# themattinthehatt/behavenet

Hardware: AMD Instinct MI355X
Metric: AE training frames/sec (128x128x1, batch 256) (higher is better)
Workload: dtype f32; 1 GPU; configs[1]: conv AE default arch, 1x128x128 f32 frames resident in HBM, 12 latents, batch 256 (chunks 200+56), fwd+bwd+Adam(amsgrad)

## Files before the change

behavenet_amd/_hip.py:

```python

import ctypes
import os

import torch

_LIB_NAME = 'libbehavenet_hip.so'
_LIB_PATH = os.environ.get('BN_HIP_LIB') or os.path.join(
    os.path.dirname(os.path.abspath(__file__)), _LIB_NAME)
_lib = None

ACT_NONE, ACT_LRELU, ACT_SIGMOID = 0, 1, 2

PROF_NONE, PROF_CONV_FWD, PROF_CONV_BWD_D, PROF_CONV_BWD_W = 0, 1, 2, 3
PROF_CONVT_FWD, PROF_CONVT_BWD_D, PROF_CONVT_BWD_W, PROF_ADAM = 4, 5, 6, 7
PROF_LINEAR_FWD, PROF_LINEAR_BWD = 8, 9

_c_int, _c_float, _c_size_t, _c_void_p = ctypes.c_int, ctypes.c_float, ctypes.c_size_t, ctypes.c_void_p

_CONV_GEOM = [_c_int] * 12
_ACT_WS = [_c_int, _c_float, _c_void_p, _c_size_t, _c_void_p]

OP_CONV_FWD, OP_CONV_BWD_D, OP_CONV_BWD_W = 1, 2, 3
OP_CONVT_FWD, OP_CONVT_BWD_D, OP_CONVT_BWD_W = 4, 5, 6

# ... 30 lines not shown
    'bn_batchnorm_act_bwd': (
        _c_int, [_c_void_p] * 9 + [_c_int] * 6 + [_c_float, _c_void_p, _c_size_t, _c_void_p]),
    'bn_batchnorm_moment': (_c_int, [_c_void_p] * 3 + [_c_int] * 3 + [_c_void_p, _c_size_t, _c_void_p]),
    'bn_batchnorm_bwd_reduce': (
        _c_int, [_c_void_p] * 7 + [_c_int] * 4 + [_c_float, _c_void_p, _c_size_t, _c_void_p]),
    'bn_batchnorm_bwd_apply': (
        _c_int, [_c_void_p] * 9 + [_c_int] * 3 + [_c_float, _c_int, _c_float, _c_void_p]),
    'bn_maxpool2d_fwd': (_c_int, [_c_void_p] * 3 + [_c_int] * 9 + [_c_void_p]),
    'bn_maxpool2d_bwd': (_c_int, [_c_void_p] * 3 + [_c_int] * 9 + [_c_void_p]),
    'bn_maxpool2d_act_fwd': (_c_int, [_c_void_p] * 3 + [_c_int] * 4 + [ctypes.c_float, _c_void_p]),
    'bn_conv2d_pool2_act_fwd': (_c_int, [_c_void_p] * 5 + _CONV_GEOM + [_c_int, _c_float, _c_void_p]),
    'bn_conv2d_pool2_act_ok': (_c_int, _CONV_GEOM),
    'bn_conv2d_pool2_bwd_weight_ws_bytes': (_c_size_t, _CONV_GEOM),
    'bn_conv2d_pool2_bwd_weight': (
        _c_int, [_c_void_p] * 6 + _CONV_GEOM + [_c_int, _c_float, _c_int, _c_void_p, _c_size_t, _c_void_p]),
    'bn_maxpool2d_act_bwd': (_c_int, [_c_void_p] * 4 + [_c_int] * 4 + [ctypes.c_float, _c_void_p]),
    'bn_maxunpool2d_fwd': (_c_int, [_c_void_p] * 3 + [_c_int] * 3 + [_c_void_p]),
    'bn_maxunpool2d_fwd_k2': (_c_int, [_c_void_p] * 3 + [_c_int] * 3 + [_c_void_p]),
    'bn_maxunpool2d_bwd': (_c_int, [_c_void_p] * 3 + [_c_int] * 3 + [_c_void_p]),
    'bn_act_fwd': (_c_int, [_c_void_p] * 2 + [_c_size_t, _c_int, _c_float, _c_void_p]),
    'bn_act_bwd': (_c_int, [_c_void_p] * 3 + [_c_size_t, _c_int, _c_float, _c_void_p]),
    'bn_linear_ws_bytes': (_c_size_t, [_c_int] * 3),
    'bn_linear_fwd': (_c_int, [_c_void_p] * 4 + [_c_int] * 3 + [_c_void_p, _c_size_t, _c_void_p]),
    'bn_linear_bwd': (
        _c_int, [_c_void_p] * 5 + [_c_int, _c_float, _c_void_p, _c_void_p, _c_int] +
        [_c_int] * 3 + [_c_void_p, _c_size_t, _c_void_p]),
    'bn_sqerr_frame_sums': (_c_int, [_c_void_p] * 4 + [_c_int, _c_size_t, _c_void_p]),
    'bn_sqerr_bwd': (_c_int, [_c_void_p] * 4 + [_c_size_t, _c_float, _c_void_p, _c_void_p]),
    'bn_convT2d_fwd_sqerr_parts': (_c_int, _CONV_GEOM),
    'bn_convT2d_fwd_sqerr_ws_bytes': (_c_size_t, _CONV_GEOM + [_c_int]),
    'bn_convT2d_fwd_sqerr': (
        _c_int, [_c_void_p] * 8 + _CONV_GEOM + [_c_int, _c_float, _c_void_p, _c_size_t, _c_void_p]),
    'bn_scale_frames': (_c_int, [_c_void_p] * 4 + [_c_int, _c_size_t, _c_void_p]),
    'bn_reduce_sum': (_c_int, [_c_void_p] * 2 + [_c_size_t, _c_float, _c_void_p]),
    'bn_reparam_fwd': (_c_int, [_c_void_p] * 4 + [_c_size_t, _c_void_p]),
    'bn_kl_rows': (_c_int, [_c_void_p] * 3 + [_c_int, _c_int, _c_void_p]),
    'bn_reparam_bwd': (_c_int, [_c_void_p] * 4 + [_c_size_t, _c_void_p]),
    'bn_kl_bwd': (_c_int, [_c_void_p] * 4 + [_c_size_t, _c_float, _c_void_p, _c_void_p]),
    'bn_decomposed_kl_fwd': (_c_int, [_c_void_p] * 7 + [_c_int, _c_int, _c_void_p]),
    'bn_decomposed_kl_bwd': (_c_int, [_c_void_p] * 9 + [_c_int, _c_int, _c_void_p]),
    'bn_psvae_head_fwd': (_c_int, [_c_void_p] * 14 + [_c_int] * 3 + [_c_void_p]),
    'bn_psvae_head_combine': (
        _c_int, [_c_void_p] * 4 + [_c_int] + [_c_float] * 3 + [_c_int] + [_c_void_p] * 3),
    'bn_psvae_head_bwd': (
        _c_int, [_c_void_p] * 3 + [_c_int] + [_c_void_p] * 10 + [_c_float] + [_c_void_p] * 5 +
        [_c_int] * 4 + [_c_void_p]),
    'bn_adam_amsgrad_step': (
        _c_int, [_c_void_p] * 5 + [_c_size_t] + [_c_float] * 5 + [_c_int, _c_void_p]),
    'bn_u8_to_unit_float': (_c_int, [_c_void_p] * 2 + [_c_size_t, _c_void_p]),
    'bn_prof_select': (_c_int, [_c_int] * 3),
    'bn_prof_select_nth': (_c_int, [_c_int] * 4),
    'bn_prof_read': (_c_int, [ctypes.POINTER(ctypes.c_double), ctypes.POINTER(ctypes.c_long)]),
    'bn_prof_read_main': (_c_int, [ctypes.POINTER(ctypes.c_double), ctypes.POINTER(ctypes.c_long)]),
    'bn_prof_set_bracket': (_c_int, [_c_int]),
    'bn_prof_kernel_name': (ctypes.c_char_p, []),
    'bn_prof_dispatch_overhead_us': (ctypes.c_double, [_c_int, _c_void_p]),
}


class HipLibraryError(RuntimeError):
    pass


def lib_path():
    return _LIB_PATH

# ... 427 lines not shown

def convT2d_fwd_sqerr(x, w, b, target, mask, geom, act, slope, want_xhat):
    N, Ci, Hi, Wi, Co, R, S, st, ct, cl, Ho, Wo = geom
    lib = load()
    P = lib.bn_convT2d_fwd_sqerr_parts(*geom)
    if P <= 0:
        raise HipLibraryError('bn_convT2d_fwd_sqerr_parts: bad geometry %s' % (geom,))
    xhat = torch.empty((N, Co, Ho, Wo), dtype=torch.float32, device=x.device) if want_xhat \
        else None
    dpre = torch.empty((N, Co, Ho, Wo), dtype=torch.float32, device=x.device)
    part = torch.empty((N, P), dtype=torch.float32, device=x.device)
    nbytes = lib.bn_convT2d_fwd_sqerr_ws_bytes(*geom, int(want_xhat))
    ws = None
    if nbytes:
        ws = _arena(x.device, nbytes, 'fwd_sqerr')
    _check(lib.bn_convT2d_fwd_sqerr(
        _ptr(x, 'x'), _ptr(w, 'w'), _ptr(b, 'b', allow_none=True), _ptr(target, 'target'),
        _ptr(mask, 'mask', allow_none=True), _ptr(xhat, 'xhat', allow_none=True),
        _ptr(dpre, 'dpre'), _ptr(part, 'part'), *geom, act, slope, ws, nbytes, _stream()),
        'bn_convT2d_fwd_sqerr')
    return xhat, dpre, part


def scale_frames(t, frame_scale, group_scale=None, group_of_frame=None):
    N = t.shape[0]
    _check(load().bn_scale_frames(
        _ptr(t, 't'), _ptr(frame_scale, 'frame_scale'),
        _ptr(group_scale, 'group_scale', allow_none=True),
        _ptr(group_of_frame, 'group_of_frame', dtype=torch.int32, allow_none=True),
        N, t.numel() // N, _stream()), 'bn_scale_frames')
    return t


def reduce_sum(t, scale=1.0, out=None):
    if out is None:
        out = torch.empty((), dtype=torch.float32, device=t.device)
    _check(load().bn_reduce_sum(_ptr(t, 'in'), _ptr(out, 'out'), t.numel(), float(scale),
                                _stream()), 'bn_reduce_sum')
    return out


def reparam_fwd(mu, logvar, eps):
    z = torch.empty_like(mu)
    _check(load().bn_reparam_fwd(
        _ptr(mu, 'mu'), _ptr(logvar, 'logvar'), _ptr(eps, 'eps'), _ptr(z, 'z'), mu.numel(),
        _stream()), 'bn_reparam_fwd')
    return z


def kl_rows(mu, logvar):
    N, D = mu.shape
    out = torch.empty((N,), dtype=torch.float32, device=mu.device)
    _check(load().bn_kl_rows(_ptr(mu, 'mu'), _ptr(logvar, 'logvar'), _ptr(out, 'kl_rows'), N, D,
                             _stream()), 'bn_kl_rows')
    return out


DECOMPOSED_KL_MAX_D = 64


def _check_dkl_width(D):
    if D > DECOMPOSED_KL_MAX_D:
        raise ValueError('decomposed KL: %d latent dimensions, the kernels serve at most %d'
                         % (D, DECOMPOSED_KL_MAX_D))


# ... 224 lines not shown
```

behavenet_amd/csrc/bn_fast.h:

```cpp
#pragma once
#include "bn_common.h"

struct BnFastPlan {
    bool supported;
    const char* kernel_name;
    size_t ws_bytes;
    int variant;
    int a, b, c, d;
};

BnFastPlan bn_fast_down_plan(const BnGeom& g);
BnFastPlan bn_fast_up_plan(const BnGeom& g);
BnFastPlan bn_fast_wgrad_plan(const BnGeom& g);

int bn_launch_down_fast(const BnFastPlan& plan, const float* big, const float* w,
                        const float* bias, float* out, const float* dact_src, const BnGeom& g,
                        int act, int dact, float slope, void* ws, hipStream_t st);
int bn_launch_up_fast(const BnFastPlan& plan, const float* small, const float* w,
                      const float* bias, float* out, const float* dact_src, const BnGeom& g,
                      int act, int dact, float slope, void* ws, hipStream_t st);
int bn_launch_wgrad_fast(const BnFastPlan& plan, const float* small, const float* big, float* dw,
                         const BnGeom& g, int accumulate, void* ws, hipStream_t st,
                         float* db = nullptr, int bias_side = 0, bool* bias_done = nullptr);

// ... 20 lines not shown
                     const BnGeom& g, int accumulate, void* ws, hipStream_t st, float* db,
                     int bias_side, bool* bias_done);

BnFastPlan bn_s5_up_plan(const BnGeom& g);
BnFastPlan bn_s5_wgrad_plan(const BnGeom& g);
int bn_launch_up_s5(const float* small, const float* w, const float* bias, float* out,
                    const float* dact_src, const BnGeom& g, int act, int dact, float slope,
                    hipStream_t st);
int bn_launch_wgrad_s5(const float* small, const float* big, float* dw, const BnGeom& g,
                       int accumulate, hipStream_t st);

BnFastPlan bn_edge_wgrad_plan(const BnGeom& g);
int bn_launch_edge_wgrad(const BnFastPlan& plan, const float* small, const float* big, float* dw,
                         const BnGeom& g, int accumulate, void* ws, hipStream_t st,
                         float* db = nullptr, int bias_side = 0, bool* bias_done = nullptr);
bool bn_s1c1_ok(const BnGeom& g);
int bn_launch_s1c1(const float* big, const float* w, const float* bias, float* out, const float* dact_src,
                   const BnGeom& g, int act, int dact, float slope, hipStream_t st);
bool bn_s1in1_ok(const BnGeom& g);
int bn_launch_s1in1(const float* big, const float* w, const float* bias, float* out, const float* dact_src,
                    const BnGeom& g, int act, int dact, float slope, hipStream_t st);
BnFastPlan bn_edge_down_plan(const BnGeom& g);
const char* bn_edge_down_kernel_name(const BnGeom& g, int act, bool has_dact, bool u8);
const char* bn_edge_up_kernel_name(const BnGeom& g, bool loss);
int bn_launch_edge_down(const float* big, const float* w, const float* bias, float* out,
                        const float* dact_src, const BnGeom& g, int act, int dact, float slope,
                        hipStream_t st, const unsigned char* u8 = nullptr);
BnFastPlan bn_edge_up_plan(const BnGeom& g);
int bn_launch_edge_up(const float* small, const float* w, const float* bias, float* out,
                      const BnGeom& g, int act, float slope, hipStream_t st,
                      const float* target = nullptr, const float* mask = nullptr,
                      float* dpre = nullptr, float* partial = nullptr);
int bn_edge_up_parts_per_frame(const BnGeom& g);

bool bn_qgemm_supported(const BnGeom& g);
size_t bn_qgemm_ws_bytes(int role, const BnGeom& g);
int bn_launch_qgemm_down(const float* big, const float* w, const float* bias, float* out,
                         const float* dact_src, const BnGeom& g, int act, int dact, float slope,
                         void* ws, hipStream_t st);
int bn_launch_qgemm_up(const float* small, const float* w, const float* bias, float* out,
                       const float* dact_src, const BnGeom& g, int act, int dact, float slope,
                       void* ws, hipStream_t st);
int bn_launch_qgemm_wgrad(const float* small, const float* big, float* dw, const BnGeom& g,
                          int accumulate, void* ws, hipStream_t st);

bool bn_qg2_up_supported(const BnGeom& g, int act, int dact);
int bn_launch_qg2_up(const float* small, const float* w, const float* bias, float* out,
                     const float* dact_src, const BnGeom& g, int act, int dact, float slope,
                     hipStream_t st);
bool bn_qg2_wgrad_supported(const BnGeom& g);
int bn_launch_qg2_wgrad(const float* small, const float* big, float* dw, const BnGeom& g,
                        int accumulate, float* db, int bias_side, hipStream_t st);

bool bn_s5win_supported(const BnGeom& g);
size_t bn_s5win_ws_bytes(int role, const BnGeom& g);
int bn_launch_s5win_down(const float* big, const float* w, const float* bias, float* out,
                         const float* dact_src, const BnGeom& g, int act, int dact, float slope,
                         void* ws, hipStream_t st);
int bn_launch_s5win_up(const float* small, const float* w, const float* bias, float* out,
                       const float* dact_src, const BnGeom& g, int act, int dact, float slope,
                       hipStream_t st);
int bn_launch_s5win_wgrad(const float* small, const float* big, float* dw, const BnGeom& g,
                          int accumulate, hipStream_t st);

int bn_launch_split_epilogue(const float* part, const float* bias, float* out, const float* dact_src,
                             size_t total, int splits, int C, int npix, int act, int dact, float slope,
// ... 2 lines not shown
```

behavenet_amd/csrc/bn_launch.h:

```cpp
#pragma once
#include "bn_common.h"

struct GemmArgs {
    const float* A; long sai, sak;
    const float* B; long sbk, sbj;
    float* C; long sci, scj;
    int M, N, K;
    const float* bias_j;
    const float* dact_src;
    int dact; float slope;
    int accumulate;
    float* part;
    int kslice;
};

int bn_launch_down_generic(const float* big, const float* w, const float* bias, float* out,
                           const float* dact_src, const BnGeom& g, int act, int dact, float slope,
                           hipStream_t st);
int bn_launch_up_generic(const float* small, const float* w, const float* bias, float* out,
                         const float* dact_src, const BnGeom& g, int act, int dact, float slope,
                         hipStream_t st);
int bn_launch_wgrad_generic(const float* small, const float* big, float* dw, const BnGeom& g,
                            int accumulate, hipStream_t st);
size_t bn_channel_sum_ws_bytes(int N, int C, int npix);
int bn_launch_channel_sum(const float* t, float* db, int N, int C, int npix, int accumulate,
                          void* ws, size_t ws_bytes, hipStream_t st);

int bn_launch_gemm(const GemmArgs& a, hipStream_t st, void* ws = nullptr, size_t ws_bytes = 0);
size_t bn_gemm_ws_bytes(int M, int N, int K);
int bn_launch_col_sum(const float* dy, float* db, int M, int N, int accumulate, hipStream_t st);
int bn_launch_linear_jobs(const GemmArgs* g0, const GemmArgs* g1, const float* dy, float* db, int M,
                          int N, int accumulate, void* ws, size_t ws_bytes, hipStream_t st);
size_t bn_linear_jobs_ws_bytes(int M, int N, int K);

int bn_launch_act_fwd(const float* x, float* y, size_t n, int act, float slope, hipStream_t st);
int bn_launch_act_bwd(const float* dy, const float* y, float* dpre, size_t n, int act, float slope,
                      hipStream_t st);
int bn_launch_sqerr_frame_sums(const float* pred, const float* target, const float* mask,
                               float* frame_sums, int N, size_t D, hipStream_t st);
int bn_launch_sqerr_bwd(const float* pred, const float* target, const float* mask, float* dpred,
                        size_t n, float scale, const float* gscale, hipStream_t st);
int bn_launch_scale_frames(float* t, const float* frame_scale, const float* group_scale,
                           const int* group_of_frame, int N, size_t D, hipStream_t st);
int bn_launch_reduce_sum(const float* in, float* out, size_t n, float scale, hipStream_t st);
int bn_launch_reparam_fwd(const float* mu, const float* logvar, const float* eps, float* z,
                          size_t n, hipStream_t st);
int bn_launch_kl_rows(const float* mu, const float* logvar, float* kl_rows, int N, int D,
                      hipStream_t st);
int bn_launch_reparam_bwd(const float* dz, const float* z, const float* mu, float* dlogvar,
                          size_t n, hipStream_t st);
int bn_launch_kl_bwd(const float* mu, const float* logvar, float* dmu, float* dlogvar, size_t n,
                     float scale, const float* gscale, hipStream_t st);
int bn_launch_adam(float* p, const float* g, float* m, float* v, float* vmax, size_t n, float lr,
                   float b1, float b2, float eps, float wd, int step, hipStream_t st);
int bn_launch_u8_to_unit_float(const unsigned char* in, float* out, size_t n, hipStream_t st);

size_t bn_batchnorm_ws_bytes_impl(int N, int C);
int bn_launch_bn_stats(const float* x, float* mean, float* var, int N, int C, int HW, void* ws,
                       hipStream_t st);
// ... 89 lines not shown
```

behavenet_amd/csrc/capi.hip:

```cpp
#include <math.h>
#include <stdio.h>
#include <stdlib.h>
#include <string.h>
#include <hip/hip_ext.h>
#include "bn_common.h"
#include "bn_launch.h"
#include "bn_fast.h"

namespace {
struct ProfState {
    int family = BN_PROF_NONE;
    int C = 0, K = 0;
    static const int kMaxSlots = 2048;
    hipEvent_t ev[4 * kMaxSlots];
    bool taken[kMaxSlots], bracketed[kMaxSlots];
    int created = 0;
    int used = 0;
    double total_ms = 0.0, main_ms = 0.0;
    long launches = 0, main_launches = 0;
    bool bracket = true;
    int nth = -1, seen = 0;
    char kernel_name[96] = "";
} g_prof;

// ... 1551 lines not shown
    if (!x || !w || !target || !dpre || !part) return BN_E_BADARG;
    const BnGeom g = convT_geom(N, Ci, Hi, Wi, Co, R, S, stride, crop_t, crop_l, Ho, Wo);
    if (!bn_geom_ok(g)) return BN_E_BADARG;
    hipStream_t st = (hipStream_t)stream;
    if (fused_sqerr_fast(g)) {
        BnProfScope prof(BN_PROF_CONVT_FWD, g.Cs, g.Cb, bn_edge_up_kernel_name(g, true), st);
        return bn_launch_edge_up(x, w, b, xhat, g, act, slope, st, target, mask, dpre, part);
    }
    const size_t need = bn_convT2d_fwd_sqerr_ws_bytes(N, Ci, Hi, Wi, Co, R, S, stride, crop_t,
                                                      crop_l, Ho, Wo, xhat != nullptr);
    if (need && (!ws || ws_bytes < need)) return BN_E_WORKSPACE;
    const size_t n_out = (size_t)N * Co * Ho * Wo;
    const size_t conv_ws = need - (xhat ? 0 : n_out * sizeof(float));
    float* xh = xhat ? xhat : (float*)((char*)ws + conv_ws);
    int rc = run_up(BN_PROF_CONVT_FWD, x, w, b, xh, nullptr, g, act, BN_ACT_NONE, slope, ws,
                    conv_ws, st);
    if (rc) return rc;
    rc = bn_launch_sqerr_frame_sums(xh, target, mask, part, N, (size_t)Co * Ho * Wo, st);
    if (rc) return rc;
    rc = bn_launch_sqerr_bwd(xh, target, mask, dpre, n_out, 1.f, nullptr, st);
    if (rc) return rc;
    if (act != BN_ACT_NONE) rc = bn_launch_act_bwd(dpre, xh, dpre, n_out, act, slope, st);
    return rc;
}

extern "C" int bn_scale_frames(float* t, const float* frame_scale, const float* group_scale,
                               const int* group_of_frame, int N, size_t D, bn_stream_t stream) {
    if (!t || !frame_scale || N <= 0 || D == 0) return BN_E_BADARG;
    if ((group_scale == nullptr) != (group_of_frame == nullptr)) return BN_E_BADARG;
    return bn_launch_scale_frames(t, frame_scale, group_scale, group_of_frame, N, D,
                                  (hipStream_t)stream);
}

extern "C" int bn_reduce_sum(const float* in, float* out, size_t n, float scale,
                             bn_stream_t stream) {
    if (!in || !out) return BN_E_BADARG;
    return bn_launch_reduce_sum(in, out, n, scale, (hipStream_t)stream);
}

extern "C" int bn_reparam_fwd(const float* mu, const float* logvar, const float* eps, float* z,
                              size_t n, bn_stream_t stream) {
    if (!mu || !logvar || !eps || !z) return BN_E_BADARG;
    if (n == 0) return 0;
    return bn_launch_reparam_fwd(mu, logvar, eps, z, n, (hipStream_t)stream);
}

extern "C" int bn_kl_rows(const float* mu, const float* logvar, float* kl_rows, int N, int D,
                          bn_stream_t stream) {
    if (!mu || !logvar || !kl_rows || N <= 0 || D <= 0) return BN_E_BADARG;
    return bn_launch_kl_rows(mu, logvar, kl_rows, N, D, (hipStream_t)stream);
}

extern "C" int bn_reparam_bwd(const float* dz, const float* z, const float* mu, float* dlogvar,
                              size_t n, bn_stream_t stream) {
    if (!dz || !z || !mu || !dlogvar) return BN_E_BADARG;
    if (n == 0) return 0;
    return bn_launch_reparam_bwd(dz, z, mu, dlogvar, n, (hipStream_t)stream);
}

extern "C" int bn_kl_bwd(const float* mu, const float* logvar, float* dmu, float* dlogvar,
                         size_t n, float scale, const float* gscale, bn_stream_t stream) {
    if (!mu || !logvar || !dmu || !dlogvar) return BN_E_BADARG;
    if (n == 0) return 0;
    return bn_launch_kl_bwd(mu, logvar, dmu, dlogvar, n, scale, gscale, (hipStream_t)stream);
}

// ... 36 lines not shown
```

behavenet_amd/csrc/conv_edge.hip:

```cpp
#include <hip/hip_ext.h>
#include <stdlib.h>
#include "bn_common.h"
#include "bn_fast.h"
#include "bn_reduce.h"

typedef float floatx16 __attribute__((ext_vector_type(16)));

#define ED_THREADS 256
#define ED_OOB 0x7fffffff

__device__ __forceinline__ float ed_ld(__amdgpu_buffer_rsrc_t r, int byte_off) {
    return __builtin_bit_cast(float, __builtin_amdgcn_raw_buffer_load_b32(r, byte_off, 0, 0));
}

#define WC_ROWS 4
#define WC_W 64
#define WC_TPX (WC_ROWS * WC_W)
#define WC_SP (WC_TPX + 2)
#define WC_IH (2 * WC_ROWS + 3)
#define WC_RW (2 * WC_W + 4)
#define WC_KS (32 * WC_TPX / ED_THREADS)

#define WC_DECODE_GRID()                                                                    \
    int bch, bx, G;                                                                         \
    if (pair) {                                                                             \
        const int id = blockIdx.x, r = id >> 3;                                             \
        G = gridDim.x / g.Cb;                                                               \
        bch = r % g.Cb;                                                                     \
        bx = (r / g.Cb) * 8 + (id & 7);                                                     \
    } else {                                                                                \
        bch = blockIdx.y; bx = blockIdx.x; G = gridDim.x;                                   \
    }

template <int ST, bool VEC = false>
__global__ __launch_bounds__(ED_THREADS) void k_wgrad_c1(
    const float* __restrict__ small, const float* __restrict__ big, float* __restrict__ part,
// ... 1467 lines not shown
            ? launch_down_c1w<BN_ACT_LRELU>(big, w, bias, out, g, slope, st, e0, e1)
            : launch_down_c1w<BN_ACT_NONE>(big, w, bias, out, g, slope, st, e0, e1);
    if (variant == 3) variant = dact_src ? 1 : 0;
    if (variant == 2) {
        if (act == BN_ACT_LRELU && !dact_src)
            return launch_down_c1s<BN_ACT_LRELU, false, false, 4>(big, w, bias, out, nullptr, g, slope, st, e0, e1);
        if (!dact_src)
            return launch_down_c1s<BN_ACT_NONE, false, false, 4>(big, w, bias, out, nullptr, g, slope, st, e0, e1);
        return launch_down_c1s<BN_ACT_NONE, true, false, 4>(big, w, bias, out, dact_src, g, slope, st, e0, e1);
    }
    if (variant == 1) {
        if (act == BN_ACT_LRELU && !dact_src)
            return launch_down_c1s<BN_ACT_LRELU, false, false, 2>(big, w, bias, out, nullptr, g, slope, st, e0, e1);
        if (!dact_src)
            return launch_down_c1s<BN_ACT_NONE, false, false, 2>(big, w, bias, out, nullptr, g, slope, st, e0, e1);
        return launch_down_c1s<BN_ACT_NONE, true, false, 2>(big, w, bias, out, dact_src, g, slope, st, e0, e1);
    }
    const int units = g.N * (g.Hs / DC_ROWS);
    const dim3 grid(down_c1_grid(units));
    if (act == BN_ACT_LRELU && !dact_src) {
        hipExtLaunchKernelGGL((k_down_c1<BN_ACT_LRELU, false>), grid, dim3(64), 0, st, e0, e1, 0,
                              big, w, bias, out, dact_src, g, slope, units);
    } else if (act == BN_ACT_NONE && !dact_src) {
        hipExtLaunchKernelGGL((k_down_c1<BN_ACT_NONE, false>), grid, dim3(64), 0, st, e0, e1, 0,
                              big, w, bias, out, dact_src, g, slope, units);
    } else {
        hipExtLaunchKernelGGL((k_down_c1<BN_ACT_NONE, true>), grid, dim3(64), 0, st, e0, e1, 0,
                              big, w, bias, out, dact_src, g, slope, units);
    }
    BN_LAUNCH_CHECK();
    return 0;
}

#define UC_TH 8
#define UC_W 64
#define UC_PW (UC_W + 2)
#define UC_NPOS ((UC_TH + 2) * UC_PW)
#define UC_NBLK ((UC_NPOS + 31) / 32)
#define UC_DP (UC_NBLK * 32)
#define UC_LDS (25 * UC_DP * 4)

__global__ __launch_bounds__(ED_THREADS) void k_up_c1(
    const float* __restrict__ small, const float* __restrict__ w, const float* __restrict__ bias,
    float* __restrict__ out, BnGeom g, int act, float slope) {
    extern __shared__ __attribute__((aligned(16))) float dl[];
    const int tid = threadIdx.x, lane = tid & 63;
    const int wv = __builtin_amdgcn_readfirstlane(tid >> 6);
    const int li = lane & 31, kk = lane >> 5;
    const int tiles_per_frame = g.Hs / UC_TH;
    const int n = blockIdx.x / tiles_per_frame;
    const int a0 = (blockIdx.x - n * tiles_per_frame) * UC_TH;
    const int HWs = g.Hs * g.Ws;

    const __amdgpu_buffer_rsrc_t rs = __builtin_amdgcn_make_buffer_rsrc(
        (void*)small, 0, (int)((size_t)g.N * g.Cs * HWs * 4), 0x00020000);

    float av[16];
#pragma unroll
    for (int t = 0; t < 16; ++t) {
        const int c = 2 * t + kk;
        av[t] = (li < 25 && c < g.Cs) ? w[(c * g.Cb + blockIdx.y) * 25 + li] : 0.f;
    }

    for (int blk = wv; blk < UC_NBLK; blk += 4) {
        const int f = blk * 32 + li;
        const int py = f / UC_PW, px = f - py * UC_PW;
// ... 1006 lines not shown
```

behavenet_amd/csrc/conv_generic.hip:

```cpp
#include "bn_common.h"
#include "bn_launch.h"

#define GEN_THREADS 256
#define GEN_MT 8
#define GEN_MAXS 16

__global__ __launch_bounds__(GEN_THREADS) void k_down_generic(
    const float* __restrict__ big, const float* __restrict__ w, const float* __restrict__ bias,
    float* __restrict__ out, const float* __restrict__ dact_src, BnGeom g, int act, int dact,
    float slope) {
    const int pix = blockIdx.x * GEN_THREADS + threadIdx.x;
    const int npix = g.Hs * g.Ws;
    const int m0 = blockIdx.y * GEN_MT;
    const int n = blockIdx.z;
    if (pix >= npix) return;
    const int p = pix / g.Ws, q = pix - p * g.Ws;
    const int RS = g.R * g.S;
    float acc[GEN_MT];
#pragma unroll
    for (int j = 0; j < GEN_MT; ++j) acc[j] = 0.f;

    const int h0 = p * g.stride - g.pt, w0 = q * g.stride - g.pl;
    for (int c = 0; c < g.Cb; ++c) {
        const float* bp = big + ((size_t)n * g.Cb + c) * g.Hb * g.Wb;
// ... 192 lines not shown
    for (int n = n_beg; n < n_end; ++n) {
        const float* tp = t + ((size_t)n * C + c) * npix;
        if (vec) {
            const float4* t4 = reinterpret_cast<const float4*>(tp);
            for (int i = threadIdx.x; i < (npix >> 2); i += GEN_THREADS) {
                const float4 v = t4[i];
                acc += (v.x + v.y) + (v.z + v.w);
            }
        } else {
            for (int i = threadIdx.x; i < npix; i += GEN_THREADS) acc += tp[i];
        }
    }
    const float s = bn_block_reduce_256(acc, red);
    if (threadIdx.x == 0) part[(size_t)c * S + sp] = s;
}

__global__ __launch_bounds__(64) void k_channel_sum_final(const float* __restrict__ part, float* __restrict__ db,
                                                          int C, int S, int accumulate) {
    const int c = blockIdx.x;
    float v = 0.f;
    for (int s = threadIdx.x; s < S; s += 64) v += part[(size_t)c * S + s];
#pragma unroll
    for (int off = 32; off > 0; off >>= 1) v += __shfl_xor(v, off, 64);
    if (threadIdx.x == 0) db[c] = accumulate ? db[c] + v : v;
}

static int channel_sum_splits(int N, int C, int npix) {
    if ((long)N * npix < 8192) return 1;
    int s = 1024 / C;
    if (s > 256) s = 256;
    if (s > N) s = N;
    return s < 1 ? 1 : s;
}

size_t bn_channel_sum_ws_bytes(int N, int C, int npix) {
    const int s = channel_sum_splits(N, C, npix);
    return s > 1 ? (size_t)C * s * sizeof(float) : 0;
}

int bn_launch_channel_sum(const float* t, float* db, int N, int C, int npix, int accumulate,
                          void* ws, size_t ws_bytes, hipStream_t st) {
    const int S = channel_sum_splits(N, C, npix);
    if (S > 1 && ws && ws_bytes >= (size_t)C * S * sizeof(float)) {
        hipLaunchKernelGGL(k_channel_sum_part, dim3(C, S), dim3(GEN_THREADS), 0, st, t, (float*)ws,
                           N, C, npix, S);
        BN_LAUNCH_CHECK();
        hipLaunchKernelGGL(k_channel_sum_final, dim3(C), dim3(64), 0, st,
                           (const float*)ws, db, C, S, accumulate);
        BN_LAUNCH_CHECK();
        return 0;
    }
    hipLaunchKernelGGL(k_channel_sum, dim3(C), dim3(GEN_THREADS), 0, st, t, db, N, C, npix,
                       accumulate);
    BN_LAUNCH_CHECK();
    return 0;
}

#include "bn_reduce.h"
__global__ __launch_bounds__(1024) void k_sum_partials(const float* __restrict__ part,
                                                       float* __restrict__ out, int total,
                                                       int splits, int accumulate, int ab_elems,
                                                       int ntap, int row_len, int row_stride) {
    __shared__ float red[16][64];
    const int il = threadIdx.x & 63, zl = threadIdx.x >> 6;
    const int nz = blockDim.x >> 6;
    const int i = blockIdx.x * 64 + il;
// ... 66 lines not shown
```

behavenet_amd/hip_functions.py:

```python

import collections.abc
import os

import torch

from behavenet_amd import _hip

LRELU_SLOPE = 0.05

_direct_grads = False


class accumulate_into_param_grads(object):

    def __enter__(self):
        global _direct_grads
        self._prev = _direct_grads
        _direct_grads = True

    def __exit__(self, *exc):
        global _direct_grads
        _direct_grads = self._prev
        return False

# ... 360 lines not shown
            if i == 0 and h1 is not None:
                h = h1
            else:
                h = _fwd(layer, h, params[2 * i].detach(), params[2 * i + 1].detach(),
                         w5=taps[i] if taps else None)
            acts.append(h)
        if _sign_tap is not None:
            rec = _sign_tap.setdefault(id(plan), [[] for _ in plan])
            for i, layer in enumerate(plan):
                if layer.act == _hip.ACT_LRELU:
                    rec[i].append((acts[i + 1] > 0).cpu())
        ctx.plan = plan
        ctx.taps = taps
        ctx.need_dx = x.requires_grad
        ctx.param_refs = params
        _note_use(params, any(ctx.needs_input_grad[3:]))
        ctx.save_for_backward(*acts, *params[0::2])
        return h

    @staticmethod
    def backward(ctx, dout):
        plan = ctx.plan
        dout = dout.contiguous()
        top = plan[-1]
        if top.act != _hip.ACT_NONE:
            dpre = _hip.act_bwd(dout, ctx.saved_tensors[len(plan)], top.act, LRELU_SLOPE)
        else:
            dpre = dout
        dx, grads = _stack_backward(ctx, dpre, first_param=3)
        return (None, dx, None) + tuple(grads)


_DGRAD_FIRST = os.environ.get('BN_DGRAD_FIRST', '0') == '1'


def _stack_backward(ctx, dpre, first_param):
    plan = ctx.plan
    n_layers = len(plan)
    saved = ctx.saved_tensors
    acts, weights = saved[:n_layers + 1], saved[n_layers + 1:2 * n_layers + 1]
    n = dpre.shape[0]
    grads = [None] * (2 * n_layers)
    taps = getattr(ctx, 'taps', None)
    tail = []
    for i in range(n_layers - 1, -1, -1):
        layer = plan[i]
        g = layer.geom(n)
        w = weights[i]
        x_in = acts[i]
        if x_in.dtype == torch.uint8:
            x_in = _hip.u8_to_unit_float(x_in) \
                if ctx.needs_input_grad[first_param + 2 * i] else None
        need_w = ctx.needs_input_grad[first_param + 2 * i]
        need_b = ctx.needs_input_grad[first_param + 1 + 2 * i]
        dpre_below = None
        if i > 0 and min(plan[i - 1].cin, plan[i - 1].cout) <= 4 and _DGRAD_FIRST:
            dact_src, dact = acts[i], plan[i - 1].act
            bwd_data = _hip.conv2d_bwd_data if layer.kind == 'conv' else _hip.convT2d_bwd_data
            dpre_below = bwd_data(dpre, w, g, dact_src, dact, LRELU_SLOPE, w5=taps[i] if taps else None)
        if need_w:
            gw = _grad_buffer(ctx.param_refs[2 * i])
            gb = _grad_buffer(ctx.param_refs[2 * i + 1]) if need_b else None
            direct = gw is not None and (gb is not None or not need_b)
            if direct:
                dw, db = gw, gb
            else:
                dw = torch.empty_like(w)
                db = torch.empty((layer.cout,), dtype=w.dtype, device=w.device) if need_b \
                    else None
            wgrad = _hip.conv2d_bwd_weight if layer.kind == 'conv' else _hip.convT2d_bwd_weight
            side = _side_stream(w.device) if (direct and _use_side_stream) else None
            if side is not None and not ctx.need_dx and i < _tail_on_main:
                tail.append(((wgrad, x_in, dpre, dw, db, g), ctx.param_refs[2 * i:2 * i + 2]))
            elif side is not None:
                main = torch.cuda.current_stream(w.device)
                ev = torch.cuda.Event()
                ev.record(main)
                with torch.cuda.stream(side):
                    side.wait_event(ev)
                    wgrad(x_in, dpre, dw, db, g, True)
                dpre.record_stream(side)
                x_in.record_stream(side)
                _report_ready(ctx.param_refs[2 * i:2 * i + 2])
            else:
                wgrad(x_in, dpre, dw, db, g, direct)
                if direct:
                    _report_ready(ctx.param_refs[2 * i:2 * i + 2])
# ... 56 lines not shown
        top = plan[-1]
        n = h.shape[0]
        xhat, dpre, part = _hip.convT2d_fwd_sqerr(
            h, params[-2].detach(), params[-1].detach(), target, mask, top.geom(n), top.act,
            LRELU_SLOPE, bool(want_xhat))
        if _sign_tap is not None:
            rec = _sign_tap.setdefault(id(plan), [[] for _ in plan])
            for i, layer in enumerate(plan[:-1]):
                if layer.act == _hip.ACT_LRELU:
                    rec[i].append((acts[i + 1] > 0).cpu())
        out = torch.empty((len(bounds),), dtype=torch.float32, device=x.device)
        for c, ((beg, end), sc) in enumerate(zip(bounds, scales)):
            _hip.reduce_sum(part[beg:end], float(sc), out=out[c:c + 1])
        ctx.plan = plan
        ctx.taps = taps
        ctx.need_dx = x.requires_grad
        ctx.param_refs = params
        ctx.bounds, ctx.scales = list(bounds), [float(sc) for sc in scales]
        ctx.consumed = False
        _note_use(params, any(ctx.needs_input_grad[7:]))
        ctx.save_for_backward(*acts, dpre, *params[0::2])
        if xhat is not None:
            ctx.mark_non_differentiable(xhat)
        return out, xhat

    @staticmethod
    def backward(ctx, g, _g_xhat):
        if ctx.consumed:
            raise RuntimeError('ConvStackSqErrFn: backward twice (dL/dpre is scaled in place)')
        ctx.consumed = True
        n_layers = len(ctx.plan)
        dpre = ctx.saved_tensors[n_layers]
        fs, ci = _frame_scales(dpre.shape[0], ctx.bounds, ctx.scales, dpre.device)
        _hip.scale_frames(dpre, fs, g.contiguous(), ci)
        dx, grads = _stack_backward(ctx, dpre, first_param=7)
        return (None, dx, None, None, None, None, None) + tuple(grads)


def conv_stack_sq_err(plan, x, params, target, mask, bounds, scales, want_xhat=False):
    return ConvStackSqErrFn.apply(plan, x, target, mask, tuple(bounds), tuple(scales),
                                  bool(want_xhat), *params)


class FusedPixelLoss(object):

    def __init__(self, x_hat, chunk_terms, kind, bounds):
        self.x_hat = x_hat
        self.chunk_terms = chunk_terms
        self.kind = kind
        self.bounds = list(bounds)


_DEVICE_CONSTANTS = {}


def device_constant(values, device):
    key = (tuple(float(v) for v in values), str(device))
    t = _DEVICE_CONSTANTS.get(key)
    if t is None:
        if len(_DEVICE_CONSTANTS) > 256:
            _DEVICE_CONSTANTS.clear()
        t = torch.tensor(key[0], dtype=torch.float32, device=device)
        _DEVICE_CONSTANTS[key] = t
    return t


def pixel_loss_scales(kind, bounds, per_frame, chunk_sizes=None):
    sizes = chunk_sizes if chunk_sizes is not None else [end - beg for beg, end in bounds]
# ... 736 lines not shown
```

include/behavenet_hip.h:

```cpp
#ifndef BEHAVENET_HIP_H
#define BEHAVENET_HIP_H

#include <stddef.h>

#ifdef __cplusplus
extern "C" {
#endif

#define BN_E_BADARG   (-1)
#define BN_E_SHAPE    (-2)
#define BN_E_WORKSPACE (-3)

#define BN_ACT_NONE    0
#define BN_ACT_LRELU   1
#define BN_ACT_SIGMOID 2

typedef void* bn_stream_t;

int         bn_version(void);
const char* bn_build_arch(void);
const char* bn_error_string(int code);

#define BN_OP_CONV_FWD    1
#define BN_OP_CONV_BWD_D  2
// ... 133 lines not shown
                         float* log_qz, float* lse, float* terms, int N, int D,
                         bn_stream_t stream);
int bn_decomposed_kl_bwd(const float* z, const float* mu, const float* logvar,
                         const float* log_qz, const float* lse, const float* g3, float* dz,
                         float* dmu, float* dlogvar, int N, int D, bn_stream_t stream);

int bn_psvae_head_fwd(const float* y, const float* w, const float* logvar, const float* eps,
                      const float* Dw, const float* Db, const float* labels, const float* lmask,
                      float* z, float* z_u, float* lv_u, float* yhat, float* row_sq,
                      float* row_kl, int N, int L, int U, bn_stream_t stream);
int bn_psvae_head_combine(const float* row_sq, const float* row_kl, const float* dkl3,
                          const int* bounds, int n_chunks, float alpha, float kl, float beta,
                          int L, float* T, float* cols5, bn_stream_t stream);
int bn_psvae_head_bwd(const float* dz, const float* gT, const int* bounds, int n_chunks,
                      const float* y, const float* logvar, const float* eps, const float* yhat,
                      const float* labels, const float* lmask, const float* Dw, const float* gz_u,
                      const float* gmu_u, const float* glv_u, float alpha, float* dy, float* dw,
                      float* dlogvar, float* dDw, float* dDb, int accumulate, int N, int L, int U,
                      bn_stream_t stream);

int bn_convT2d_fwd_sqerr_parts(int N, int Ci, int Hi, int Wi, int Co, int R, int S, int stride,
                               int crop_t, int crop_l, int Ho, int Wo);
size_t bn_convT2d_fwd_sqerr_ws_bytes(int N, int Ci, int Hi, int Wi, int Co, int R, int S,
                                     int stride, int crop_t, int crop_l, int Ho, int Wo,
                                     int with_xhat);
int bn_convT2d_fwd_sqerr(const float* x, const float* w, const float* b, const float* target,
                         const float* mask, float* xhat, float* dpre, float* part,
                         int N, int Ci, int Hi, int Wi, int Co, int R, int S, int stride,
                         int crop_t, int crop_l, int Ho, int Wo, int act, float slope,
                         void* ws, size_t ws_bytes, bn_stream_t stream);
int bn_scale_frames(float* t, const float* frame_scale, const float* group_scale,
                    const int* group_of_frame, int N, size_t D, bn_stream_t stream);

int bn_adam_amsgrad_step(float* p, const float* g, float* m, float* v, float* vmax, size_t n,
                         float lr, float beta1, float beta2, float eps, float weight_decay,
                         int step, bn_stream_t stream);

size_t bn_conv2d_fwd_u8_ws_bytes(int N, int C, int H, int W, int K, int R, int S, int stride,
                                 int pad_t, int pad_l, int P, int Q, int act);
int bn_conv2d_fwd_u8(const unsigned char* x, const float* w, const float* b, float* y,
                     int N, int C, int H, int W, int K, int R, int S, int stride,
                     int pad_t, int pad_l, int P, int Q, int act, float slope,
                     void* ws, size_t ws_bytes, bn_stream_t stream);

int bn_u8_to_unit_float(const unsigned char* in, float* out, size_t n, bn_stream_t stream);

#define BN_PROF_NONE        0
#define BN_PROF_CONV_FWD    1
#define BN_PROF_CONV_BWD_D  2
#define BN_PROF_CONV_BWD_W  3
#define BN_PROF_CONVT_FWD   4
#define BN_PROF_CONVT_BWD_D 5
#define BN_PROF_CONVT_BWD_W 6
#define BN_PROF_ADAM        7
#define BN_PROF_LINEAR_FWD  8
#define BN_PROF_LINEAR_BWD  9
int bn_prof_select(int family, int C, int K);
int bn_prof_select_nth(int family, int C, int K, int nth);
int bn_prof_read(double* total_ms, long* launches);
int bn_prof_read_main(double* total_ms, long* launches);
int bn_prof_set_bracket(int on);
const char* bn_prof_kernel_name(void);
double bn_prof_dispatch_overhead_us(int iters, bn_stream_t stream);

#ifdef __cplusplus
}
// ... 3 lines not shown
```

Before: 58800 frames/s.

## Fuse final convT backward: frame scaling, dgrad, activation grad, wgrad and bias sum

After: 59330 frames/s, median of 6. Within noise of the previous version (+0.9%).

```diff
diff --git a/behavenet_amd/_hip.py b/behavenet_amd/_hip.py
--- a/behavenet_amd/_hip.py
+++ b/behavenet_amd/_hip.py
@@ -86,6 +86,10 @@
     'bn_convT2d_fwd_sqerr': (
         _c_int, [_c_void_p] * 8 + _CONV_GEOM + [_c_int, _c_float, _c_void_p, _c_size_t, _c_void_p]),
     'bn_scale_frames': (_c_int, [_c_void_p] * 4 + [_c_int, _c_size_t, _c_void_p]),
+    'bn_convT2d_bwd_fused_kernel': (ctypes.c_char_p, _CONV_GEOM),
+    'bn_convT2d_bwd_fused_ws_bytes': (_c_size_t, _CONV_GEOM),
+    'bn_convT2d_bwd_fused': (
+        _c_int, [_c_void_p] * 9 + _CONV_GEOM + [_c_int, _c_float, _c_int, _c_void_p, _c_size_t, _c_void_p]),
     'bn_reduce_sum': (_c_int, [_c_void_p] * 2 + [_c_size_t, _c_float, _c_void_p]),
     'bn_reparam_fwd': (_c_int, [_c_void_p] * 4 + [_c_size_t, _c_void_p]),
     'bn_kl_rows': (_c_int, [_c_void_p] * 3 + [_c_int, _c_int, _c_void_p]),
@@ -579,6 +583,31 @@
     return t
 
 
+_bwd_fused_kernels = {}
+
+
+def convT2d_bwd_fused_kernel(geom):
+    key = (_generic_epoch,) + tuple(geom)
+    if key not in _bwd_fused_kernels:
+        name = load().bn_convT2d_bwd_fused_kernel(*geom)
+        _bwd_fused_kernels[key] = name.decode() if name else None
+    return _bwd_fused_kernels[key]
+
+
+def convT2d_bwd_fused(x, dy, w, dw, db, geom, frame_scale, group_scale, group_of_frame, dact, slope,
+                      accumulate):
+    N, Ci, Hi, Wi = geom[:4]
+    dx = torch.empty((N, Ci, Hi, Wi), dtype=torch.float32, device=dy.device)
+    nbytes = load().bn_convT2d_bwd_fused_ws_bytes(*geom)
+    ws = _arena(dy.device, nbytes, 'bwd_fused') if nbytes else None
+    _check(load().bn_convT2d_bwd_fused(
+        _ptr(x, 'x'), _ptr(dy, 'dy'), _ptr(w, 'w'), _ptr(dx, 'dx'), _ptr(dw, 'dw'), _ptr(db, 'db'),
+        _ptr(frame_scale, 'frame_scale'), _ptr(group_scale, 'group_scale', allow_none=True),
+        _ptr(group_of_frame, 'group_of_frame', dtype=torch.int32, allow_none=True), *geom, dact, slope,
+        int(accumulate), ws, nbytes, _stream()), 'bn_convT2d_bwd_fused')
+    return dx
+
+
 def reduce_sum(t, scale=1.0, out=None):
     if out is None:
         out = torch.empty((), dtype=torch.float32, device=t.device)
diff --git a/behavenet_amd/csrc/bn_fast.h b/behavenet_amd/csrc/bn_fast.h
--- a/behavenet_amd/csrc/bn_fast.h
+++ b/behavenet_amd/csrc/bn_fast.h
@@ -76,6 +76,11 @@
                       const float* target = nullptr, const float* mask = nullptr,
                       float* dpre = nullptr, float* partial = nullptr);
 int bn_edge_up_parts_per_frame(const BnGeom& g);
+bool bn_edge_bwd_fused_ok(const BnGeom& g);
+size_t bn_edge_bwd_fused_ws_bytes(const BnGeom& g);
+int bn_launch_edge_bwd_fused(const float* dpre, const float* w, const float* h, float* dh, float* dw,
+                             float* db, const float* fs, const float* gs, const int* gi, const BnGeom& g,
+                             float slope, int accumulate, void* ws, hipStream_t st);
 
 bool bn_qgemm_supported(const BnGeom& g);
 size_t bn_qgemm_ws_bytes(int role, const BnGeom& g);
diff --git a/behavenet_amd/csrc/bn_launch.h b/behavenet_amd/csrc/bn_launch.h
--- a/behavenet_amd/csrc/bn_launch.h
+++ b/behavenet_amd/csrc/bn_launch.h
@@ -25,6 +25,8 @@
 size_t bn_channel_sum_ws_bytes(int N, int C, int npix);
 int bn_launch_channel_sum(const float* t, float* db, int N, int C, int npix, int accumulate,
                           void* ws, size_t ws_bytes, hipStream_t st);
+int bn_launch_channel_sum_g4(const float* g4, float* db, int N, int npix, int accumulate, float* part,
+                             hipStream_t st);
 
 int bn_launch_gemm(const GemmArgs& a, hipStream_t st, void* ws = nullptr, size_t ws_bytes = 0);
 size_t bn_gemm_ws_bytes(int M, int N, int K);
diff --git a/behavenet_amd/csrc/capi.hip b/behavenet_amd/csrc/capi.hip
--- a/behavenet_amd/csrc/capi.hip
+++ b/behavenet_amd/csrc/capi.hip
@@ -1607,6 +1607,39 @@
                                   (hipStream_t)stream);
 }
 
+static bool bwd_fused_served(const BnGeom& g) { return bn_geom_ok(g) && !force_generic() && bn_edge_bwd_fused_ok(g); }
+
+extern "C" const char* bn_convT2d_bwd_fused_kernel(int N, int Ci, int Hi, int Wi, int Co, int R, int S,
+                                                   int stride, int crop_t, int crop_l, int Ho, int Wo) {
+    const BnGeom g = convT_geom(N, Ci, Hi, Wi, Co, R, S, stride, crop_t, crop_l, Ho, Wo);
+    return bwd_fused_served(g) ? "k_bwd_c1f" : nullptr;
+}
+
+extern "C" size_t bn_convT2d_bwd_fused_ws_bytes(int N, int Ci, int Hi, int Wi, int Co, int R, int S,
+                                                int stride, int crop_t, int crop_l, int Ho, int Wo) {
+    const BnGeom g = convT_geom(N, Ci, Hi, Wi, Co, R, S, stride, crop_t, crop_l, Ho, Wo);
+    return bwd_fused_served(g) ? bn_edge_bwd_fused_ws_bytes(g) : 0;
+}
+
+extern "C" int bn_convT2d_bwd_fused(const float* x, const float* dy, const float* w, float* dx, float* dw,
+                                    float* db, const float* frame_scale, const float* group_scale,
+                                    const int* group_of_frame, int N, int Ci, int Hi, int Wi, int Co, int R,
+                                    int S, int stride, int crop_t, int crop_l, int Ho, int Wo, int dact,
+                                    float slope, int accumulate, void* ws, size_t ws_bytes, bn_stream_t stream) {
+    TapsHintDrop hint_drop;
+    if (!x || !dy || !w || !dx || !dw || !db || !frame_scale) return BN_E_BADARG;
+    if ((group_scale == nullptr) != (group_of_frame == nullptr)) return BN_E_BADARG;
+    const BnGeom g = convT_geom(N, Ci, Hi, Wi, Co, R, S, stride, crop_t, crop_l, Ho, Wo);
+    if (!bn_geom_ok(g)) return BN_E_BADARG;
+    if (!bwd_fused_served(g) || dact != BN_ACT_LRELU || !aligned16_all(x, dy, w, dx)) return BN_E_SHAPE;
+    const size_t need = bn_edge_bwd_fused_ws_bytes(g);
+    if (!ws || ws_bytes < need) return BN_E_WORKSPACE;
+    hipStream_t st = (hipStream_t)stream;
+    BnProfScope prof(BN_PROF_CONVT_BWD_D, g.Cb, g.Cs, "k_bwd_c1f", st);
+    return bn_launch_edge_bwd_fused(dy, w, x, dx, dw, db, frame_scale, group_scale, group_of_frame, g, slope,
+                                    accumulate, ws, st);
+}
+
 extern "C" int bn_reduce_sum(const float* in, float* out, size_t n, float scale,
                              bn_stream_t stream) {
     if (!in || !out) return BN_E_BADARG;
diff --git a/behavenet_amd/csrc/conv_edge.hip b/behavenet_amd/csrc/conv_edge.hip
--- a/behavenet_amd/csrc/conv_edge.hip
+++ b/behavenet_amd/csrc/conv_edge.hip
@@ -2,6 +2,7 @@
 #include <stdlib.h>
 #include "bn_common.h"
 #include "bn_fast.h"
+#include "bn_launch.h"
 #include "bn_reduce.h"
 
 typedef float floatx16 __attribute__((ext_vector_type(16)));
@@ -1535,6 +1536,186 @@
     return 0;
 }
 
+#define FB_TR (2 * WC_ROWS + 3)
+#define FB_TILE (FB_TR * DC_RW)
+#define FB_HS 33
+#define FB_SLAB (32 * FB_HS)
+#define FB_NLD ((FB_TR * 32 + ED_THREADS - 1) / ED_THREADS)
+#define FB_LDS (FB_TILE + 4 * FB_SLAB)
+
+__global__ __launch_bounds__(ED_THREADS, 2) void k_bwd_c1f(
+    const float* __restrict__ dpre, const float* __restrict__ w, float* __restrict__ out,
+    const float* __restrict__ h, const float* __restrict__ fs, const float* __restrict__ gs,
+    const int* __restrict__ gi, float* __restrict__ part, float* __restrict__ g4, BnGeom g, float slope,
+    int n_stages, int spf) {
+    __shared__ __attribute__((aligned(16))) float lds[FB_LDS];
+    float* tile = lds;
+    const int tid = threadIdx.x, lane = tid & 63;
+    const int wv = __builtin_amdgcn_readfirstlane(tid >> 6);
+    const int li = lane & 31, kk = lane >> 5;
+    float* hs = lds + FB_TILE + wv * FB_SLAB;
+    const int G = gridDim.x, bx = blockIdx.x;
+    const int HWb = g.Hb * g.Wb, PQ = g.Hs * g.Ws;
+
+    const __amdgpu_buffer_rsrc_t rb = __builtin_amdgcn_make_buffer_rsrc(
+        (void*)dpre, 0, (int)((size_t)g.N * HWb * 4), 0x00020000);
+    const __amdgpu_buffer_rsrc_t ro = __builtin_amdgcn_make_buffer_rsrc(
+        (void*)out, 0, (int)((size_t)g.N * g.Cs * PQ * 4), 0x00020000);
+    const __amdgpu_buffer_rsrc_t rd = __builtin_amdgcn_make_buffer_rsrc(
+        (void*)h, 0, (int)((size_t)g.N * g.Cs * PQ * 4), 0x00020000);
+
+    for (int e = tid; e < FB_TR * 8; e += ED_THREADS) {
+        const int y = e >> 3, c = e & 7;
+        tile[y * DC_RW + (c < 4 ? c : DC_X0 + 2 * DC_W + c - 4)] = 0.f;
+    }
+    const int st_lane = (4 * kk * PQ + li) * 4;
+    auto issue = [&](int st, intx4 (&tr)[FB_NLD], float (&dm)[32]) {
+        const int n = st / spf;
+        const int p0 = (st - n * spf) * WC_ROWS;
+        const int hb0 = 2 * p0 - g.pt;
+#pragma unroll
+        for (int k = 0; k < FB_NLD; ++k) {
+            const int e = tid + ED_THREADS * k;
+            const int y = e >> 5, cg = e & 31, hb = hb0 + y;
+            const bool ok = e < FB_TR * 32 && hb >= 0 && hb < g.Hb;
+            tr[k] = __builtin_amdgcn_raw_buffer_load_b128(rb, ok ? ((n * g.Hb + hb) * g.Wb + 4 * cg) * 4 : ED_OOB,
+                                                          0, 0);
+        }
+        const int row_off = ((n * g.Cs * g.Hs + p0 + wv) * DC_W) * 4;
+#pragma unroll
+        for (int qh = 0; qh < 2; ++qh)
+#pragma unroll
+            for (int e = 0; e < 16; ++e) {
+                const int chb = (e & 3) + 8 * (e >> 2);
+                const bool ok = chb + 4 * kk < g.Cs;
+                dm[16 * qh + e] = __builtin_bit_cast(float, __builtin_amdgcn_raw_buffer_load_b32(
+                    rd, ok ? st_lane : ED_OOB, row_off + (chb * PQ + 32 * qh) * 4, 0));
+            }
+    };
+
+    float wv_[13];
+#pragma unroll
+    for (int t = 0; t < 13; ++t) {
+        const int tap = 2 * t + kk;
+        wv_[t] = (tap < 25 && li < g.Cs) ? w[li * 25 + tap] : 0.f;
+    }
+    const float* ar = tile + DC_X0 - g.pl + 2 * li + (2 * wv) * DC_RW;
+    const float* arA = ar + kk;
+    const float* arB = ar + kk * (DC_RW - 4);
+    const int tap = li < 25 ? li : 0;
+    const int tr_ = tap / 5, ts = tap - tr_ * 5;
+    const float* hA = hs + li * FB_HS + kk;
+    const float* pB = tile + (2 * wv + tr_) * DC_RW + DC_X0 - g.pl + ts + 2 * kk;
+    floatx16 accw[2];
+#pragma unroll
+    for (int h2 = 0; h2 < 2; ++h2)
+#pragma unroll
+        for (int e = 0; e < 16; ++e) accw[h2][e] = 0.f;
+
+    intx4 tr[FB_NLD];
+    float dm[32];
+    int st = bx;
+    if (st < n_stages) issue(st, tr, dm);
+#pragma unroll 1
+    for (; st < n_stages; st += G) {
+        const int n = st / spf;
+        const int p0 = (st - n * spf) * WC_ROWS;
+        float sc = fs[n];
+        if (gs) sc *= gs[gi[n]];
+        __syncthreads();
+#pragma unroll
+        for (int k = 0; k < FB_NLD; ++k) {
+            const int e = tid + ED_THREADS * k;
+            if (e >= FB_TR * 32) continue;
+            const int y = e >> 5, cg = e & 31;
+            floatx4e v = __builtin_bit_cast(floatx4e, tr[k]);
+            v.x *= sc; v.y *= sc; v.z *= sc; v.w *= sc;
+            *reinterpret_cast<floatx4e*>(tile + y * DC_RW + DC_X0 + 4 * cg) = v;
+            if (y >= 1 && y <= 2 * WC_ROWS)
+                g4[(size_t)n * (HWb >> 2) + (2 * p0 - g.pt + y) * (g.Wb >> 2) + cg] = (v.x + v.y) + (v.z + v.w);
+        }
+        float d[32];
+#pragma unroll
+        for (int e = 0; e < 32; ++e) d[e] = dm[e];
+        __syncthreads();
+        if (st + G < n_stages) issue(st + G, tr, dm);
+
+        floatx16 acc[2];
+#pragma unroll
+        for (int qh = 0; qh < 2; ++qh)
+#pragma unroll
+            for (int e = 0; e < 16; ++e) acc[qh][e] = 0.f;
+#pragma unroll
+        for (int t = 0; t < 13; ++t) {
+            const int t0 = ((2 * t) / 5) * DC_RW + (2 * t) % 5;
+            const float* at = ((2 * t) % 5 == 4 && t != 12) ? arB : arA;
+#pragma unroll
+            for (int qh = 0; qh < 2; ++qh)
+                acc[qh] = __builtin_amdgcn_mfma_f32_32x32x2f32(wv_[t], at[t0 + 64 * qh], acc[qh], 0, 0, 0);
+        }
+        const int row_off = ((n * g.Cs * g.Hs + p0 + wv) * DC_W) * 4;
+#pragma unroll
+        for (int qh = 0; qh < 2; ++qh) {
+#pragma unroll
+            for (int e = 0; e < 16; ++e) {
+                const int chb = (e & 3) + 8 * (e >> 2);
+                const int so = row_off + (chb * PQ + 32 * qh) * 4;
+                const bool ok = chb + 4 * kk < g.Cs;
+                float v = acc[qh][e];
+                v *= d[16 * qh + e] > 0.f ? 1.f : slope;
+                __builtin_amdgcn_raw_buffer_store_b32(__builtin_bit_cast(int, v), ro, ok ? st_lane : ED_OOB, so, 0);
+            }
+#pragma unroll
+            for (int e = 0; e < 16; ++e) hs[((e & 3) + 8 * (e >> 2) + 4 * kk) * FB_HS + li] = d[16 * qh + e];
+            const float* pq = pB + 64 * qh;
+#pragma unroll
+            for (int j = 0; j < 16; ++j)
+                accw[j & 1] = __builtin_amdgcn_mfma_f32_32x32x2f32(hA[2 * j], pq[4 * j], accw[j & 1], 0, 0, 0);
+        }
+    }
+
+    __syncthreads();
+    float* red = lds;
+#pragma unroll
+    for (int e = 0; e < 16; ++e) red[(wv * 16 + e) * 64 + lane] = accw[0][e] + accw[1][e];
+    __syncthreads();
+    if (wv == 0 && li < 25) {
+#pragma unroll
+        for (int e = 0; e < 16; ++e) {
+            const float v = (red[e * 64 + lane] + red[(16 + e) * 64 + lane]) +
+                            (red[(32 + e) * 64 + lane] + red[(48 + e) * 64 + lane]);
+            const int a = (e & 3) + 8 * (e >> 2) + 4 * kk;
+            if (a < g.Cs) part[(size_t)bx * (g.Cs * 25) + a * 25 + li] = v;
+        }
+    }
+}
+
+bool bn_edge_bwd_fused_ok(const BnGeom& g) {
+    return g.R == 5 && g.S == 5 && g.stride == 2 && g.Cb == 1 && g.Cs <= 32 && g.CsS == 0 && g.KV == 0 &&
+           g.K0 == 0 && g.Ws == DC_W && g.Wb == 2 * g.Ws && g.Hb == 2 * g.Hs && (g.Hs % WC_ROWS) == 0 &&
+           g.pt == 1 && g.pl == 1 && g.N * g.Cb >= 128 && (size_t)g.N * g.Cs * g.Hs * g.Ws * 4 < 0x7fffffffull;
+}
+
+size_t bn_edge_bwd_fused_ws_bytes(const BnGeom& g) {
+    const size_t part = (size_t)wgrad_c1_grid(g) * g.Cs * 25, grp = (size_t)g.N * g.Hb * g.Wb / 4;
+    return (part + grp + 1024) * sizeof(float);
+}
+
+int bn_launch_edge_bwd_fused(const float* dpre, const float* w, const float* h, float* dh, float* dw,
+                             float* db, const float* fs, const float* gs, const int* gi, const BnGeom& g,
+                             float slope, int accumulate, void* ws, hipStream_t st) {
+    const int G = wgrad_c1_grid(g), spf = g.Hs / WC_ROWS, n_stages = g.N * spf;
+    float* part = (float*)ws;
+    float* grp = part + (size_t)G * g.Cs * 25;
+    float* bias_part = grp + (size_t)g.N * g.Hb * g.Wb / 4;
+    BN_LAUNCH_MAIN(k_bwd_c1f, dim3(G), dim3(ED_THREADS), 0, st, dpre, w, dh, h, fs, gs, gi, part, grp, g, slope,
+                   n_stages, spf);
+    BN_LAUNCH_CHECK();
+    int rc = bn_launch_sum_partials(part, dw, g.Cs * 25, G, accumulate, 0, 0, st, 25, g.Cb * 25);
+    if (rc) return rc;
+    return bn_launch_channel_sum_g4(grp, db, g.N, g.Hb * g.Wb, accumulate, bias_part, st);
+}
+
 #define UC_TH 8
 #define UC_W 64
 #define UC_PW (UC_W + 2)
diff --git a/behavenet_amd/csrc/conv_generic.hip b/behavenet_amd/csrc/conv_generic.hip
--- a/behavenet_amd/csrc/conv_generic.hip
+++ b/behavenet_amd/csrc/conv_generic.hip
@@ -248,6 +248,42 @@
     if (s > N) s = N;
     return s < 1 ? 1 : s;
 }
+
+__global__ __launch_bounds__(GEN_THREADS) void k_channel_sum_part_g4(
+    const float* __restrict__ g4, float* __restrict__ part, int N, int per, int S) {
+    __shared__ float red[4];
+    const int sp = blockIdx.x;
+    const int n_beg = (int)((long)sp * N / S), n_end = (int)((long)(sp + 1) * N / S);
+    float acc = 0.f;
+    for (int n = n_beg; n < n_end; ++n) {
+        const float* src = g4 + (size_t)n * per;
+        for (int i0 = threadIdx.x; i0 < per; i0 += 16 * GEN_THREADS) {
+            float v[16];
+#pragma unroll
+            for (int k = 0; k < 16; ++k) {
+                const int i = i0 + k * GEN_THREADS;
+                v[k] = i < per ? src[i] : 0.f;
+            }
+#pragma unroll
+            for (int k = 0; k < 16; ++k)
+                if (i0 + k * GEN_THREADS < per) acc += v[k];
+        }
+    }
+    const float s = bn_block_reduce_256(acc, red);
+    if (threadIdx.x == 0) part[sp] = s;
+}
+
+int bn_launch_channel_sum_g4(const float* g4, float* db, int N, int npix, int accumulate, float* part,
+                             hipStream_t st) {
+    const int S = channel_sum_splits(N, 1, npix), per = npix >> 2;
+    if (S <= 1 || S > 1024 || (npix & 3) || per < GEN_THREADS) return BN_E_SHAPE;
+    hipLaunchKernelGGL(k_channel_sum_part_g4, dim3(S), dim3(GEN_THREADS), 0, st, g4, part, N, per, S);
+    BN_LAUNCH_CHECK();
+    hipLaunchKernelGGL(k_channel_sum_final, dim3(1), dim3(64), 0, st, (const float*)part, db, 1, S, accumulate);
+    BN_LAUNCH_CHECK();
+    return 0;
+}
+
 
 size_t bn_channel_sum_ws_bytes(int N, int C, int npix) {
     const int s = channel_sum_splits(N, C, npix);
diff --git a/behavenet_amd/hip_functions.py b/behavenet_amd/hip_functions.py
--- a/behavenet_amd/hip_functions.py
+++ b/behavenet_amd/hip_functions.py
@@ -416,9 +416,27 @@
 
 
 _DGRAD_FIRST = os.environ.get('BN_DGRAD_FIRST', '0') == '1'
-
-
-def _stack_backward(ctx, dpre, first_param):
+_FUSED_TOP_BWD = os.environ.get('BN_FUSED_TOP_BWD', '1') != '0'
+
+
+def _top_bwd_fused(ctx, n, first_param):
+    if not _FUSED_TOP_BWD:
+        return False
+    if _direct_grads and not _single_pass:
+        return False
+    plan = ctx.plan
+    i = len(plan) - 1
+    if i == 0 or plan[i].kind != 'convT' or plan[i - 1].act != _hip.ACT_LRELU:
+        return False
+    if not (ctx.needs_input_grad[first_param + 2 * i] and ctx.needs_input_grad[first_param + 1 + 2 * i]):
+        return False
+    saved = ctx.saved_tensors
+    if any(t.data_ptr() % 16 for t in (saved[i], saved[i + 1], saved[len(plan) + 1 + i])):
+        return False
+    return _hip.convT2d_bwd_fused_kernel(plan[i].geom(n)) is not None
+
+
+def _stack_backward(ctx, dpre, first_param, top_scale=None):
     plan = ctx.plan
     n_layers = len(plan)
     saved = ctx.saved_tensors
@@ -437,6 +455,22 @@
                 if ctx.needs_input_grad[first_param + 2 * i] else None
         need_w = ctx.needs_input_grad[first_param + 2 * i]
         need_b = ctx.needs_input_grad[first_param + 1 + 2 * i]
+        if top_scale is not None and i == n_layers - 1:
+            gw = _grad_buffer(ctx.param_refs[2 * i])
+            gb = _grad_buffer(ctx.param_refs[2 * i + 1])
+            direct = gw is not None and gb is not None
+            if direct:
+                dw, db = gw, gb
+            else:
+                dw = torch.empty_like(w)
+                db = torch.empty((layer.cout,), dtype=w.dtype, device=w.device)
+            dpre = _hip.convT2d_bwd_fused(x_in, dpre, w, dw, db, g, *top_scale, plan[i - 1].act, LRELU_SLOPE,
+                                          direct)
+            if direct:
+                _report_ready(ctx.param_refs[2 * i:2 * i + 2])
+            else:
+                grads[2 * i], grads[2 * i + 1] = dw, db
+            continue
         dpre_below = None
         if i > 0 and min(plan[i - 1].cin, plan[i - 1].cout) <= 4 and _DGRAD_FIRST:
             dact_src, dact = acts[i], plan[i - 1].act
@@ -559,8 +593,11 @@
         n_layers = len(ctx.plan)
         dpre = ctx.saved_tensors[n_layers]
         fs, ci = _frame_scales(dpre.shape[0], ctx.bounds, ctx.scales, dpre.device)
-        _hip.scale_frames(dpre, fs, g.contiguous(), ci)
-        dx, grads = _stack_backward(ctx, dpre, first_param=7)
+        if _top_bwd_fused(ctx, dpre.shape[0], first_param=7):
+            dx, grads = _stack_backward(ctx, dpre, first_param=7, top_scale=(fs, g.contiguous(), ci))
+        else:
+            _hip.scale_frames(dpre, fs, g.contiguous(), ci)
+            dx, grads = _stack_backward(ctx, dpre, first_param=7)
         return (None, dx, None, None, None, None, None) + tuple(grads)
 
 
diff --git a/include/behavenet_hip.h b/include/behavenet_hip.h
--- a/include/behavenet_hip.h
+++ b/include/behavenet_hip.h
@@ -189,6 +189,16 @@
 int bn_scale_frames(float* t, const float* frame_scale, const float* group_scale,
                     const int* group_of_frame, int N, size_t D, bn_stream_t stream);
 
+const char* bn_convT2d_bwd_fused_kernel(int N, int Ci, int Hi, int Wi, int Co, int R, int S, int stride,
+                                        int crop_t, int crop_l, int Ho, int Wo);
+size_t bn_convT2d_bwd_fused_ws_bytes(int N, int Ci, int Hi, int Wi, int Co, int R, int S, int stride,
+                                     int crop_t, int crop_l, int Ho, int Wo);
+int bn_convT2d_bwd_fused(const float* x, const float* dy, const float* w, float* dx, float* dw, float* db,
+                         const float* frame_scale, const float* group_scale, const int* group_of_frame,
+                         int N, int Ci, int Hi, int Wi, int Co, int R, int S, int stride, int crop_t,
+                         int crop_l, int Ho, int Wo, int dact, float slope, int accumulate, void* ws,
+                         size_t ws_bytes, bn_stream_t stream);
+
 int bn_adam_amsgrad_step(float* p, const float* g, float* m, float* v, float* vmax, size_t n,
                          float lr, float beta1, float beta2, float eps, float weight_decay,
                          int step, bn_stream_t stream);
```
